# VatsalSy/gerris-fft-particles

Measured on AMD Instinct MI355X. Metric: Mcell-steps/s (projection+advection), 3D 256^3 uniform, higher is better.
Workload: dtype f64; 1 GPU; 3-D periodic Taylor-Green, 256^3 per GPU, default projection/advection parameters (SURVEY 8d config C); relax_mode=exact, parallelism=1 box, rccl_world_size=0

## Files before the change

### gerris-fft-particles_amd/csrc/domain.hip

```cpp
#include "gfship_internal.hpp"

namespace gfship {

static thread_local char g_error[1024] = "";

void set_error (const char * fmt, ...)
{
  va_list ap;
  va_start (ap, fmt);
  vsnprintf (g_error, sizeof (g_error), fmt, ap);
  va_end (ap);
}

int hip_fail (hipError_t e, const char * what, const char * file, int line)
{
  set_error ("HIP error %d (%s) in %s at %s:%d", (int) e, hipGetErrorString (e), what, file, line);
  return e == hipErrorOutOfMemory ? GFSHIP_ENOMEM : GFSHIP_EHIP;
}

Field * get_field (gfship_domain * dom, gfship_field f)
{
  if (!dom || f < 0 || (size_t) f >= dom->fields.size () || !dom->fields[f].used) {
    set_error ("invalid field handle %d", f);
    return nullptr;
// ... 162 lines not shown
  dom->gather_ctx = ctx;
  dom->lat_rank = rank; dom->lat_n = nboxes;
  for (int c = 0; c < 3; c++) dom->lat_b[c] = lattice[c];
  return GFSHIP_OK;
}

int gfship_domain_path_counts (gfship_domain * dom, unsigned long long * lattice_cycles,
			       unsigned long long * fused_mpi_launches)
{
  GFSHIP_CHECK (dom != nullptr, GFSHIP_EINVAL, "null domain");
  if (lattice_cycles) *lattice_cycles = dom->n_lattice_cycles;
  if (fused_mpi_launches) *fused_mpi_launches = dom->n_fused_mpi;
  return GFSHIP_OK;
}

int gfship_domain_kernel_counts (gfship_domain * dom, unsigned long long * counts, int n)
{
  GFSHIP_CHECK (dom != nullptr && counts != nullptr && n >= 0, GFSHIP_EINVAL, "null argument");
  for (int k = 0; k < n && k < GFSHIP_KC_COUNT; k++)
    counts[k] = dom->kc[k];
  return GFSHIP_OK;
}

int gfship_domain_synchronize (gfship_domain * dom)
{
  GFSHIP_CHECK (dom != nullptr, GFSHIP_EINVAL, "null domain");
  GFSHIP_HIP (hipStreamSynchronize (dom->stream));
  return GFSHIP_OK;
}

// ... 177 lines not shown
```

### gerris-fft-particles_amd/csrc/gfship_internal.hpp

```cpp
#pragma once

#include <hip/hip_runtime.h>
#include <cstdio>
#include <cstdarg>
#include <cstring>
#include <vector>
#include <deque>
#include <string>
#include <type_traits>
#include "gfship.h"
#include "switches.hpp"
#include "cell_update.hpp"

namespace gfship {

struct Layout {
  int n = 0;
  int px = 0;
  int xo = 1;
  int rows = 0;
  int dim = 3;
  long sy = 0;
  long sz = 0;
  size_t total = 0;
// ... 75 lines not shown
  size_t scratch_doubles = 0;
  double * h_pinned = nullptr;
  gfship_exchange_fn exchange = nullptr; void * exchange_ctx = nullptr;
  gfship_reduce_fn reduce = nullptr;     void * reduce_ctx = nullptr;
  bool has_external = false;
  void * comm = nullptr;
  int overlap = 0;
  int lat_rank = -1, lat_n = 0, lat_b[3] = { 1, 1, 1 };
  gfship_gather_fn gather = nullptr; void * gather_ctx = nullptr;
  double * lat_res = nullptr, * lat_xch = nullptr;
  unsigned * lat_bar = nullptr;
  size_t lat_res_doubles = 0, lat_xch_doubles = 0;
  double * gfv_send[6] = {}, * gfv_recv[6] = {};
  double src[3] = { 0., 0., 0. };
  unsigned long long n_lattice_cycles = 0, n_fused_mpi = 0;
  unsigned long long kc[GFSHIP_KC_COUNT] = {};
  bool lattice_attr_set = false;
  void * mpi_plan[GFSHIP_MAXLEVEL + 1] = {};
  gfship_field dp_cache = -1;
  int skew_resident = -1;
  int patch_resident = 0;
  bool no_fused_godunov = false;
  bool no_fused_loop = false;
  bool force_hyperplane = false;
  bool unit_weights = false;
  bool weighted = false;
  unsigned long weights_stamp = 0;
  gfship_field wf[6] = {-1, -1, -1, -1, -1, -1};
  gfship::SkewPlan skew[GFSHIP_MAXLEVEL + 1];
  double diff_w[GFSHIP_MAXLEVEL + 1] = {};
// ... 106 lines not shown
			   double * u, const double * rhs, const double * dia);
int launch_residual (gfship_domain * dom, int level, const double * u, const double * rhs,
		     const double * dia, double * res);
int launch_residual_weighted (gfship_domain * dom, int level, const double * u, const double * rhs,
			      const double * dia, double * res);
int launch_poisson_weights (gfship_domain * dom, double * const alpha[3]);
int launch_diffusion_weights (gfship_domain * dom, double * const D[3], double cdt);
int alloc_weights (gfship_domain * dom);
RelaxOp weighted_op (gfship_domain * dom, int level);
int launch_restrict (gfship_domain * dom, unsigned dimension, int level_coarse, double * v_coarse,
		     const double * v_fine);
int launch_prolongate (gfship_domain * dom, int level_coarse, const double * v_coarse,
		       double * v_fine);
int launch_correct (gfship_domain * dom, int level, double * u, const double * dp);
int launch_fill (gfship_domain * dom, int level, double * a, double value);
int launch_residual_norm (gfship_domain * dom, int level, const double * u, const double * rhs,
			  const double * dia, double * res, double scale, double weight,
			  double * out , bool dia_zero = false);
int launch_norm_async (gfship_domain * dom, int level, const double * a, double scale, double weight);
int launch_norm (gfship_domain * dom, int level, const double * a, double scale, double weight,
		 double out[5] );

int launch_face_interp_un (gfship_domain * dom, double * const u[3], double * const un[3]);
int launch_divergence (gfship_domain * dom, double * const un[3], double * div, double dt);
int launch_correct_un (gfship_domain * dom, const double * p, double * const un[3], double dt);
int launch_centered_gradient (gfship_domain * dom, const double * p, double * const g[3]);
int launch_correct_centered (gfship_domain * dom, double * const u[3], double * const g[3], double dt);
int launch_correct_centered_coarse (gfship_domain * dom, double * const u[3], double * const g[3],
				    double dt, double * const uc[3]);
int launch_coarse_init_from (gfship_domain * dom, Field * const * v, int nf, int top);
int launch_coarse_init_levels (gfship_domain * dom, Field * const * v, int nf, int top, int bottom);
int launch_advected_face_values (gfship_domain * dom, const double * v, double * const u[3],
				 double * const un[3], double dt, int use_centered, int gradient,
// ... 81 lines not shown
```

### gerris-fft-particles_amd/csrc/poisson.hip

```cpp
#include "gfship_internal.hpp"
#include <cmath>
#include <cfloat>
#include <cstdlib>

using namespace gfship;

namespace gfship {

static bool weighted_pipelinable (gfship_domain * dom, unsigned dimension, int level)
{
  return dom->relax_mode == GFSHIP_RELAX_EXACT && dimension == 3 && dom->dim == 3 &&
    skew_supported (dom, level) && !dom->force_hyperplane;
}

static bool weighted_pipelined (gfship_domain * dom, unsigned dimension, int level)
{
  return dom->sw.weighted_pipelined && weighted_pipelinable (dom, dimension, level);
}

static int relax_level (gfship_domain * dom, unsigned dimension, int level, double omega,
			Field * u, Field * rhs, Field * dia)
{
  u->zero[level] = false;
  if (dom->weighted) {
// ... 383 lines not shown
extern "C" {

int gfship_poisson_cycle (gfship_domain * dom, gfship_multilevel_params * p,
			  gfship_field u, gfship_field rhs, gfship_field dia, gfship_field res)
{
  GFSHIP_CHECK (dom != nullptr, GFSHIP_EINVAL, "null domain");
  int r = before_write (dom);
  if (r) return r;
  return poisson_cycle (dom, p, u, rhs, dia, res, 1., nullptr);
}

int gfship_poisson_solve (gfship_domain * dom, gfship_multilevel_params * par,
			  gfship_field lhs, gfship_field rhs, gfship_field res,
			  gfship_field dia, double dt)
{
  GFSHIP_CHECK (dom && par, GFSHIP_EINVAL, "null argument");
  Field * U = get_field (dom, lhs), * R = get_field (dom, rhs), * D = get_field (dom, dia),
    * S = get_field (dom, res);
  if (!U || !R || !D || !S) return GFSHIP_EINVAL;
  GFSHIP_CHECK (dom->unit_weights, GFSHIP_EINVAL, "call gfship_poisson_coefficients first");
  { int r = before_write (dom); if (r) return r; }
  int r;
  const int L = dom->depth;
  if ((r = coarse_flush (dom, U, L, true))) return r;
  unsigned minlevel = par->minlevel;
  par->depth = L;
  par->niter = 0;

  bool deferred = par->nitermin >= 1 && par->nitermax >= 1;
  if (deferred) {
    const Layout & Ly = dom->lay[L];
    double size = 1./Ly.n;
    S->zero[L] = false;
    if (dom->weighted) {
      if ((r = launch_residual_weighted (dom, L, U->lev[L], R->lev[L], D->lev[L], S->lev[L]))) return r;
      if ((r = launch_norm_async (dom, L, S->lev[L], 1.*size*size, 1.))) return r;
    }
    else if ((r = launch_residual_norm (dom, L, U->lev[L], R->lev[L], D->lev[L], S->lev[L], 1.*size*size,
					1., nullptr, D->zero[L])))
      return r;
  }
  else {
    if ((r = residual_and_norm (dom, dt, U, R, D, S, &par->residual))) return r;
    par->residual_before = par->residual;
  }

  double res_max_before = par->residual.infty;

  while (par->niter < par->nitermin ||
	 (par->residual.infty > par->tolerance && par->niter < par->nitermax)) {
    if ((r = poisson_cycle (dom, par, lhs, rhs, dia, res, dt, &par->residual))) {
      if (deferred) {
	deferred = false;
	double s0[5];
	if (hipStreamSynchronize (dom->stream) == hipSuccess) {
	  memcpy (s0, dom->h_pinned + 8, sizeof (s0));
	  if (norm_residual_finish (dom, dt, s0, &par->residual_before) == GFSHIP_OK)
	    par->residual = par->residual_before;
	}
	else
// ... 13 lines not shown
      break;
    if (par->residual.infty > res_max_before/1.1 && par->minlevel < par->depth)
      par->minlevel++;
    res_max_before = par->residual.infty;
    par->niter++;
  }

  par->minlevel = minlevel;
  if (r == GFSHIP_OK)
    r = skew_check_error (dom);
  if (r == GFSHIP_OK)
    r = lattice_check_error (dom);
  return r;
}

int gfship_time_relax (gfship_domain * dom, unsigned d, int level, gfship_field u,
		       gfship_field rhs, gfship_field dia, int reps, double * ms_per_sweep)
{
  Field * U = get_field (dom, u), * R = get_field (dom, rhs), * D = get_field (dom, dia);
  if (!U || !R || !D || !ms_per_sweep || reps <= 0) return GFSHIP_EINVAL;
  GFSHIP_CHECK (level >= 0 && level <= dom->depth, GFSHIP_EINVAL, "level %d out of range", level);
  int r;
  if (dom->relax_mode == GFSHIP_RELAX_EXACT && d == 3 && skew_supported (dom, level) &&
      !dom->force_hyperplane) {
    U->zero[level] = false;
    r = skew_time_sweeps (dom, level, U, R->lev[level], D->lev[level], D->zero[level], reps,
			  ms_per_sweep);
    if (r == GFSHIP_OK && dom->sw.skew_stats)
      skew_dump_stats (dom, level);
    return r;
// ... 43 lines not shown
```

### gerris-fft-particles_amd/csrc/poisson_kernels.hip

```cpp
#include "gfship_internal.hpp"
#include "cell_loop.hpp"
#include "relax_skew.hpp"
#include <algorithm>
#include <cstdlib>

namespace gfship {

template <int DIM, int OP>
__device__ __forceinline__ double relax_value (const double * __restrict__ u, long c, long sy, long sz,
					       double rhs, double dia, unsigned dimension,
					       double omega, double w, double h2, const W6 * wf = nullptr)
{
  return cell_update<DIM, OP> (kind_weights<OP> (w, ArrayW { wf, c }), ArrayU { u, c, sy, sz }, rhs, dia, u + c,
			       dimension, omega, h2);
}

__device__ __forceinline__ double relax_value_six (const double * __restrict__ u, long c, long sy, long sz,
						    double rhs)
{
  return cell_update_six (ArrayU { u, c, sy, sz }, rhs);
}

template <int DIM, int OP>
__global__ void __launch_bounds__(256)
// ... 1036 lines not shown
  }
  GFSHIP_HIP (hipGetLastError ());
  return GFSHIP_OK;
}

template <int DIM>
__global__ void __launch_bounds__(256)
residual_kernel (Layout L, const double * __restrict__ u, const double * __restrict__ rhs,
		 const double * __restrict__ dia, double * __restrict__ res)
{
  CELL_LOOP_PROLOGUE (L);
  const FaceSums s = face_sums<DIM> (UnitW {}, ArrayU { u, c, L.sy, L.sz }, dia[c]);
  res[c] = residual_close (s.a, s.b, rhs[c], u[c]);
}

template <bool NORM>
__global__ void residual_norm2_kernel (Layout L, const double * __restrict__ u, const double * __restrict__ rhs,
				       const double * __restrict__ dia, double * __restrict__ res, double inv,
				       double weight, double * __restrict__ partial);

int launch_residual (gfship_domain * dom, int level, const double * u, const double * rhs,
		     const double * dia, double * res)
{
  const Layout & L = dom->lay[level];
  dim3 grid, block;
  cell_grid (L, &grid, &block);
  const bool pairs = dom->sw.residual_pairs;
  if (dom->dim == 3 && L.n >= 64) dom->kc[pairs ? GFSHIP_KC_RESIDUAL_PAIRS : GFSHIP_KC_RESIDUAL_SCALAR]++;
  if (dom->dim == 3 && L.n >= 64 && pairs) {
    const long nitems = (long) L.n*L.n*(L.n/2);
    long nb = (nitems + 255)/256;
    if (nb > 4096) nb = 4096;
    hipLaunchKernelGGL (residual_norm2_kernel<false>, dim3 ((int) nb), dim3 (256), 0, dom->stream, L, u, rhs,
			dia, res, 1., 1., nullptr);
    GFSHIP_HIP (hipGetLastError ());
    return GFSHIP_OK;
  }
  with_bools ([&] (auto D3) {
    hipLaunchKernelGGL (residual_kernel<decltype (D3)::value ? 3 : 2>, grid, block, 0, dom->stream, L, u, rhs, dia, res);
  }, dom->dim == 3);
  GFSHIP_HIP (hipGetLastError ());
  return GFSHIP_OK;
}

template <int DIM>
__global__ void __launch_bounds__(256)
residual_weighted_kernel (Layout L, const double * __restrict__ u, const double * __restrict__ rhs,
			  const double * __restrict__ dia, double * __restrict__ res, W6 wf)
{
// ... 383 lines not shown
      const FaceSums f = face_sums<DIM> (UnitW {}, ArrayU { u, c, L.sy, L.sz }, dia ? dia[c] : 0.);
      const double raw = residual_close (f.a, f.b, rhs[c], u[c]);
      res[c] = raw;
      double val = raw*inv;
      s0 += weight*val;
      val = fabs (val);
      s3 = fmax (s3, val);
      s1 += weight*val;
      s2 += weight*val*val;
      s4 += raw;
    }
  }
  block_norm_sums (s0, s1, s2, s3, s4, partial, blockIdx.x);
}

template <bool NORM>
__global__ void __launch_bounds__(256)
residual_norm2_kernel (Layout L, const double * __restrict__ u, const double * __restrict__ rhs,
		       const double * __restrict__ dia, double * __restrict__ res, double inv,
		       double weight, double * __restrict__ partial)
{
  typedef double d2 __attribute__((ext_vector_type(2)));
  const int n = L.n, half = n >> 1;
  const long nitems = (long) n*n*half;
  double s0 = 0., s1 = 0., s2 = 0., s3 = 0., s4 = 0.;
  for (long it = (long) blockIdx.x*blockDim.x + threadIdx.x; it < nitems; it += (long) gridDim.x*blockDim.x) {
    const int pr = (int) (it % half);
    const long r = it / half;
    const int j = (int) (r % n) + 1, k = (int) (r / n) + 1;
    const long c = L.idx (1 + 2*pr, j, k);
    const d2 uc = *(const d2 *) (u + c);
    const double ul = u[c - 1], ur = u[c + 2];
    const d2 ut = *(const d2 *) (u + c + L.sy), ub = *(const d2 *) (u + c - L.sy);
    const d2 uf = *(const d2 *) (u + c + L.sz), uk = *(const d2 *) (u + c - L.sz);
    const d2 rh = *(const d2 *) (rhs + c);
// ... 9 lines not shown
      a += 1.; b += 1.*uf.x;
      a += 1.; b += 1.*uk.x;
      out.x = rh.x - (b - uc.x*a);
    }
    {
      double a = di.y, b = 0.;
      a += 1.; b += 1.*ur;
      a += 1.; b += 1.*uc.x;
      a += 1.; b += 1.*ut.y;
      a += 1.; b += 1.*ub.y;
      a += 1.; b += 1.*uf.y;
      a += 1.; b += 1.*uk.y;
      out.y = rh.y - (b - uc.y*a);
    }
    *(d2 *) (res + c) = out;
    if (NORM)
#pragma unroll
    for (int e = 0; e < 2; e++) {
      const double raw = e ? out.y : out.x;
      double val = raw*inv;
      s0 += weight*val;
      val = fabs (val);
      s3 = fmax (s3, val);
      s1 += weight*val;
      s2 += weight*val*val;
      s4 += raw;
    }
  }
  if (!NORM) return;
  __shared__ double sh[5][4];
// ... 2 lines not shown
  if (lane == 0) { sh[0][w] = s0; sh[1][w] = s1; sh[2][w] = s2; sh[3][w] = s3; sh[4][w] = s4; }
  __syncthreads ();
  if (threadIdx.x == 0) {
    int nw = blockDim.x >> 6;
    double r0 = 0., r1 = 0., r2 = 0., r3 = 0., r4 = 0.;
    for (int q = 0; q < nw; q++) {
      r0 += sh[0][q]; r1 += sh[1][q]; r2 += sh[2][q]; r3 = fmax (r3, sh[3][q]); r4 += sh[4][q];
    }
    double * p = partial + 5*(size_t) blockIdx.x;
    p[0] = r0; p[1] = r1; p[2] = r2; p[3] = r3; p[4] = r4;
  }
}

int launch_residual_norm (gfship_domain * dom, int level, const double * u, const double * rhs,
			  const double * dia, double * res, double scale, double weight,
			  double * out, bool dia_zero)
{
  const Layout & L = dom->lay[level];
  if (!power_of_two (scale)) {
    int r = launch_residual (dom, level, u, rhs, dia, res);
    if (r) return r;
    return out ? launch_norm (dom, level, res, scale, weight, out) :
      launch_norm_async (dom, level, res, scale, weight);
  }
  long nrows = L.dim == 3 ? (long) L.n*L.n : L.n;
  int block = L.n >= 256 ? 256 : L.n >= 128 ? 128 : 64;
  int rn_blocks = dom->sw.rn_blocks;
  if (rn_blocks < 64 || rn_blocks > 8192) rn_blocks = 4096;
  int nblocks = (int) (nrows > rn_blocks ? rn_blocks : nrows);
  double * partial = dom->d_scratch;
  double * result = out ? dom->h_pinned : dom->h_pinned + 8;
  const bool rn_pairs = dom->sw.residual_pairs;
  if (dom->dim == 3 && L.n >= 64) dom->kc[rn_pairs ? GFSHIP_KC_RESIDUAL_PAIRS : GFSHIP_KC_RESIDUAL_SCALAR]++;
  if (dom->dim == 3 && L.n >= 64 && rn_pairs) {
    const long nitems = (long) L.n*L.n*(L.n/2);
    long nb = (nitems + 255)/256;
    nblocks = (int) (nb > rn_blocks ? rn_blocks : nb);
    hipLaunchKernelGGL (residual_norm2_kernel<true>, dim3 (nblocks), dim3 (256), 0, dom->stream, L, u,
			rhs, dia_zero ? nullptr : dia, res, 1./scale, weight, partial);
  }
  else
    with_bools ([&] (auto D3) {
      hipLaunchKernelGGL (residual_norm_kernel<decltype (D3)::value ? 3 : 2>, dim3 (nblocks), dim3 (block), 0,
			  dom->stream, L, u, rhs, dia_zero ? nullptr : dia, res, 1./scale, weight, partial);
    }, dom->dim == 3);
  hipLaunchKernelGGL (norm_final_kernel, dim3 (1), dim3 (256), 0, dom->stream,
		      partial, nblocks, result);
  GFSHIP_HIP (hipGetLastError ());
  dom->kc[GFSHIP_KC_RN_BLOCKS_LIMIT] = rn_blocks;
  if ((unsigned long long) nblocks > dom->kc[GFSHIP_KC_RN_BLOCKS_MAX])
    dom->kc[GFSHIP_KC_RN_BLOCKS_MAX] = nblocks;
  if (out) {
    GFSHIP_HIP (stream_wait_spin (dom->stream));
    memcpy (out, dom->h_pinned, 5*sizeof (double));
// ... 159 lines not shown
```

### gerris-fft-particles_amd/csrc/simulation.hip

```cpp
#include "gfship_internal.hpp"
#include <cmath>
#include <cfloat>
#include <cstdlib>

using namespace gfship;

#define G_MAXINT 2147483647

struct gfship_sim {
  gfship_domain * dom = nullptr;
  gfship_field p = -1, pmac = -1, u[3] = {-1, -1, -1}, g[3] = {-1, -1, -1}, gmac[3] = {-1, -1, -1};
  std::vector<gfship_field> tracers;
  std::vector<int> tracer_gradient;
  gfship_field un[3] = {-1, -1, -1};
  gfship_field fv[6] = {-1, -1, -1, -1, -1, -1};
  gfship_field dia = -1, div = -1, res = -1, tmp = -1;
  gfship_multilevel_params projection_params, approx_projection_params;
  gfship_advection_params advection_params;
  double t = 0., end = DBL_MAX, dtmax = DBL_MAX, tnext = 0.;
  unsigned i = 0, iend = G_MAXINT;
  double visc[3] = {0., 0., 0.};
  gfship_field alpha[3] = {-1, -1, -1};
  bool has_alpha = false;
  gfship_field viscf[3][3] = {{-1, -1, -1}, {-1, -1, -1}, {-1, -1, -1}};
// ... 120 lines not shown
}

int materialize_un (gfship_sim * s)
{
  if (!s->un_lazy) return GFSHIP_OK;
  s->un_lazy = false;
  double * uold[3], * un[3];
  ptrs3 (s, s->adv_tmp3, uold);
  ptrs3 (s, s->un, un);
  TRY (launch_face_interp_un (s->dom, uold, un));
  TRY (launch_correct_un (s->dom, leaf (s, s->p), un, s->un_lazy_dt));
  return GFSHIP_OK;
}

int mac_projection (gfship_sim * s, gfship_multilevel_params * par, double dt, gfship_field p,
		    const gfship_field g[3], bool approximate = false, bool lazy = false)
{
  gfship_domain * dom = s->dom;
  double * un[3], * gp[3], * u[3];
  ptrs3 (s, s->un, un);
  ptrs3 (s, g, gp);
  ptrs3 (s, s->u, u);
  if (s->has_alpha) {
    TRY (gfship_poisson_coefficients_alpha (dom, s->alpha));
    lazy = false;
  }
  else
    TRY (gfship_poisson_coefficients (dom));
  for (int l = 0; l <= dom->depth; l++)
    if (!dom->fields[s->dia].zero[l])
      TRY (gfship_field_fill (dom, s->dia, l, 0.));
// ... 2 lines not shown
  if (!approximate || !s->tracers.empty () || s->un_handle_given || p != s->p || !dom->sw.lazy_un)
    lazy = false;
  if (!approximate)
    TRY (materialize_un (s));
  else
    s->un_lazy = false;
  if (approximate)
    TRY (launch_face_interp_div (dom, u, lazy ? nullptr : un, leaf (s, s->div), dt));
  else if (!(s->div_ready && s->div_dt == dt)) {
    TRY (launch_divergence (dom, un, leaf (s, s->div), dt));
    dom->kc[GFSHIP_KC_DIVERGENCE_SEPARATE]++;
  }
  else
    dom->kc[GFSHIP_KC_DIVERGENCE_FUSED]++;
  s->div_ready = false;
  TRY (gfship_poisson_solve (dom, par, p, s->div, s->res, s->dia, dt));
  s->cfl_ready = false;
  bool want_max = approximate, ghosts_done = false;
  for (int c = 0; c < dom->dim; c++)
    if (has_viscosity (s, c) || dom->src[c] != 0. || s->has_srcf) want_max = false;
  if (s->has_alpha) {
    want_max = false;
    TRY (launch_project_correct_weighted (dom, leaf (s, p), un, gp, approximate ? u : nullptr, dt));
  }
  else if (lazy) {
    const int L = dom->depth;
    double * uo[3];
    for (int c = 0; c < dom->dim; c++) {
      if (s->adv_tmp3[c] < 0)
	s->adv_tmp3[c] = gfship_field_alloc (dom, -1);
      if (s->adv_tmp3[c] < 0) return s->adv_tmp3[c];
// ... 671 lines not shown
    v.push_back (get_field (dom, s->u[c]));
  for (gfship_field t : s->tracers)
    v.push_back (get_field (dom, t));
}

int gfship_sim_set_tracer_gradient (gfship_sim * s, int t, int gradient)
{
  GFSHIP_CHECK (s != nullptr, GFSHIP_EINVAL, "null simulation");
  GFSHIP_CHECK (t >= 0 && (size_t) t < s->tracers.size (), GFSHIP_EINVAL, "no tracer %d", t);
  GFSHIP_CHECK (gradient >= 0 && gradient <= 4, GFSHIP_EINVAL,
		"gradient: 0 centred, 1 van Leer, 2 minmod, 3 superbee, 4 sweby");
  s->tracer_gradient[t] = gradient;
  return GFSHIP_OK;
}

static int coarse_init (gfship_sim * s, bool u_done);

int gfship_coarse_init (gfship_sim * s)
{
  GFSHIP_CHECK (s != nullptr, GFSHIP_EINVAL, "null simulation");
  return coarse_init (s, false);
}

static int coarse_init (gfship_sim * s, bool u_done)
{
  std::vector<Field *> v;
  sim_variables (s, v);
  Field * pmac = get_field (s->dom, s->pmac);
  std::vector<Field *> now, vel;
  for (Field * F : v) {
    bool is_u = false;
    for (int c = 0; c < s->dom->dim; c++)
      if (F == get_field (s->dom, s->u[c])) is_u = true;
    if (F == pmac) F->coarse_stale = true;
    else {
      F->coarse_stale = false;
      F->coarse_valid = true;
      if (u_done && is_u) vel.push_back (F); else now.push_back (F);
    }
  }
  if (vel.empty ())
    return launch_coarse_init (s->dom, now.data (), (int) now.size ());
  TRY (launch_coarse_init_levels (s->dom, now.data (), (int) now.size (), s->dom->depth - 1, s->dom->depth - 1));
  now.insert (now.end (), vel.begin (), vel.end ());
  if (s->dom->depth >= 2)
    TRY (launch_coarse_init_levels (s->dom, now.data (), (int) now.size (), s->dom->depth - 2, 0));
  return GFSHIP_OK;
}

int gfship_sim_start (gfship_sim * s)
{
  GFSHIP_CHECK (s != nullptr, GFSHIP_EINVAL, "null simulation");
  GFSHIP_CHECK (s->advection_params.gc, GFSHIP_EUNSUPPORTED, "gc = 0 is not supported");
  TRY (bc_leaf (s, s->p));
  TRY (bc_leaf (s, s->pmac));
// ... 57 lines not shown

  {
    Field * P = get_field (dom, s->p), * PM = get_field (dom, s->pmac);
    std::swap (P->lev, PM->lev);
    int r = mac_projection (s, &s->projection_params, s->advection_params.dt/2., s->p, s->gmac);
    std::swap (P->lev, PM->lev);
    if (r != GFSHIP_OK) return r;
  }

  bool u_coarse = false, corrected = false;
  TRY (centered_velocity_advection (s, s->gmac, s->i > 0 ? gc : s->gmac, - s->advection_params.dt,
				    &corrected, &u_coarse));
  if (!corrected)
    TRY (correct_centered_velocities (s, s->i > 0 ? gc : s->gmac, - s->advection_params.dt, &u_coarse));

  TRY (coarse_init (s, u_coarse));

  TRY (mac_projection (s, &s->approx_projection_params, s->advection_params.dt, s->p, s->g, true, true));
  s->t = s->tnext;
  s->i++;

  TRY (set_timestep (s, true));
  TRY (advance_tracers (s, s->advection_params.dt));
  return GFSHIP_OK;
}

int gfship_divergence_norm (gfship_sim * s, gfship_norm * out)
{
  GFSHIP_CHECK (s && out, GFSHIP_EINVAL, "null argument");
  double * u[3];
  ptrs3 (s, s->u, u);
  TRY (launch_velocity_divergence (s->dom, u, leaf (s, s->div)));
  return gfship_norm_variable (s->dom, s->div, out);
// ... 12 lines not shown
```

### gerris-fft-particles_amd/csrc/timestep_kernels.hip

```cpp
#include "gfship_internal.hpp"
#include "cell_loop.hpp"
#include <cfloat>

namespace gfship {

#define EXT_PROLOGUE(L)							\
  int i = blockIdx.x*blockDim.x + threadIdx.x;				\
  int j = blockIdx.y;							\
  int k = (L).dim == 3 ? blockIdx.z : 0;				\
  if (i > (L).n) return;						\
  long c = (L).idx (i, j, k)

static inline void ext_grid (const Layout & L, dim3 * grid, dim3 * block)
{
  int b = L.n >= 256 ? 256 : L.n >= 128 ? 128 : 64;
  *block = dim3 (b);
  *grid = dim3 ((L.n + 1 + b - 1)/b, L.n + 1, L.dim == 3 ? L.n + 1 : 1);
}

struct Ptr3  { double * p[3]; };
struct CPtr3 { const double * p[3]; };
struct Ptr6  { double * p[6]; };
struct CPtr6 { const double * p[6]; };
struct Visc3 { double d[3]; double g[3]; };
// ... 2527 lines not shown
  for (int f = 0; f < A.nf; f++) {
    double val = 0., sa = 0.;
#pragma unroll
    for (int id = 0; id < (1 << DIM); id++) {
      int ci = 2*i - 1 + (id & 1);
      int cj = 2*j - 1 + ((id & 2) ? 0 : 1);
      int ck = DIM == 3 ? 2*k - 1 + ((id & 4) ? 0 : 1) : 0;
      double a = 1.;
      val += A.vf[f][Lf.idx (ci, cj, ck)]*a;
      sa += a;
    }
    A.vc[f][c] = val/sa;
  }
}

template <int DIM>
__global__ void __launch_bounds__(256)
velocity_divergence_kernel (Layout L, CPtr3 u, double * __restrict__ out)
{
  CELL_LOOP_PROLOGUE (L);
  const long off[3] = { 1, L.sy, L.sz };
  double h = 1./L.n;
  double div = 0.;
#pragma unroll
  for (int cc = 0; cc < DIM; cc++) {
    div += 1.*1.*face_interp (u.p[cc][c], u.p[cc][c + off[cc]]);
    div += 1.*-1.*face_interp (u.p[cc][c], u.p[cc][c - off[cc]]);
  }
  out[c] = div/(1.*h);
}
// ... 481 lines not shown

int launch_coarse_init (gfship_domain * dom, Field * const * v, int nf)
{
  return launch_coarse_init_from (dom, v, nf, dom->depth - 1);
}

int launch_coarse_init_from (gfship_domain * dom, Field * const * v, int nf, int top)
{
  return launch_coarse_init_levels (dom, v, nf, top, 0);
}

int launch_coarse_init_levels (gfship_domain * dom, Field * const * v, int nf, int top, int bottom)
{
  for (int f0 = 0; f0 < nf; f0 += 8) {
    int m = nf - f0 < 8 ? nf - f0 : 8;
    for (int l = top; l >= bottom; l--) {
      const Layout & Lc = dom->lay[l], & Lf = dom->lay[l + 1];
      CoarseArgs A;
      A.nf = m;
      for (int f = 0; f < m; f++) {
	A.vc[f] = v[f0 + f]->lev[l];
	A.vf[f] = v[f0 + f]->lev[l + 1];
	v[f0 + f]->zero[l] = false;
	v[f0 + f]->coarse_valid = true;
      }
      dim3 grid, block;
      cell_grid (Lc, &grid, &block);
      DISPATCH (dom, coarse_init_kernel, grid, block, Lc, Lf, A);
    }
  }
  return GFSHIP_OK;
}

int launch_velocity_divergence (gfship_domain * dom, double * const u[3], double * out)
{
  const Layout & L = dom->lay[dom->depth];
  dim3 grid, block;
  cell_grid (L, &grid, &block);
  DISPATCH (dom, velocity_divergence_kernel, grid, block, L, c3 (u), out);
  return GFSHIP_OK;
}

}
```

### gerris-fft-particles_amd/gfship/__init__.py

```python
import ctypes as C
import os
import sys

import numpy as np

_PKG = os.path.dirname(os.path.dirname(os.path.abspath(__file__)))
LIB_PATH = os.environ.get("GFSHIP_LIB", os.path.join(_PKG, "lib", "libgfship.so"))

SIDE_PERIODIC, SIDE_BOUNDARY, SIDE_EXTERNAL = 0, 1, 2
BC_SYMMETRY, BC_DIRICHLET, BC_NEUMANN = 0, 1, 2
RELAX_EXACT, RELAX_REDBLACK, RELAX_EXACT_HYPERPLANE, RELAX_EXACT_PER_SWEEP = 0, 1, 2, 3


class GfshipError(RuntimeError):
    pass


class Norm(C.Structure):
    _fields_ = [("bias", C.c_double), ("first", C.c_double), ("second", C.c_double),
                ("infty", C.c_double), ("w", C.c_double)]


class MultilevelParams(C.Structure):
    _fields_ = [("tolerance", C.c_double), ("nrelax", C.c_uint), ("erelax", C.c_uint),
# ... 29 lines not shown
    "gfship_field_download": (_i, [_vp, _i, _i, _pd]),
    "gfship_field_fill": (_i, [_vp, _i, _i, _d]),
    "gfship_field_device_ptr": (_vp, [_vp, _i, _i, _pi, _pi]),
    "gfship_bc": (_i, [_vp, _i, _i, _i]),
    "gfship_homogeneous_bc": (_i, [_vp, _i, _i, _i]),
    "gfship_multilevel_params_init": (None, [C.POINTER(MultilevelParams), _i]),
    "gfship_poisson_coefficients": (_i, [_vp]),
    "gfship_poisson_coefficients_alpha": (_i, [_vp, _pi]),
    "gfship_poisson_weights": (_i, [_vp, _i, _pi]),
    "gfship_relax": (_i, [_vp, _u, _i, _d, _i, _i, _i]),
    "gfship_residual": (_i, [_vp, _u, _i, _i, _i, _i, _i]),
    "gfship_norm_residual": (_i, [_vp, _d, _i, C.POINTER(Norm)]),
    "gfship_norm_variable": (_i, [_vp, _i, C.POINTER(Norm)]),
    "gfship_poisson_cycle": (_i, [_vp, C.POINTER(MultilevelParams), _i, _i, _i, _i]),
    "gfship_poisson_solve": (_i, [_vp, C.POINTER(MultilevelParams), _i, _i, _i, _i, _d]),
    "gfship_diffusion_coefficients": (_i, [_vp, _d, _d, _i, _d]),
    "gfship_diffusion_coefficients_faces": (_i, [_vp, _pi, _d, _i, _i, _d]),
    "gfship_diffusion_rhs": (_i, [_vp, _i, _i, _i, _d]),
    "gfship_diffusion_residual": (_i, [_vp, _i, _i, _i, _i]),
    "gfship_diffusion_cycle": (_i, [_vp, _u, _u, _u, _i, _i, _i, _i]),
    "gfship_diffusion": (_i, [_vp, C.POINTER(MultilevelParams), _i, _i, _i]),
    "gfship_time_relax": (_i, [_vp, _u, _i, _i, _i, _i, _i, _pd]),
    "gfship_time_relax_loop": (_i, [_vp, _i, _i, _i, _i, _u, _i, _pd, _pi]),
    "gfship_time_relax_loop_inclusive": (_i, [_vp, _i, _i, _i, _i, _u, _i, _pd, _pi, _pd]),
    "gfship_sim_create": (_i, [C.POINTER(_vp), _vp]),
    "gfship_sim_destroy": (None, [_vp]),
    "gfship_sim_variable": (_i, [_vp, _i, _i]),
    "gfship_sim_projection_params": (C.POINTER(MultilevelParams), [_vp]),
    "gfship_sim_approx_projection_params": (C.POINTER(MultilevelParams), [_vp]),
    "gfship_sim_advection_params": (C.POINTER(AdvectionParams), [_vp]),
# ... 19 lines not shown
    "gfship_approximate_projection": (_i, [_vp, C.POINTER(MultilevelParams), _d, _i, _pi]),
    "gfship_centered_velocity_advection": (_i, [_vp, _pi, _pi]),
    "gfship_correct_centered_velocities": (_i, [_vp, _pi, _d]),
    "gfship_sim_advance_time": (_i, [_vp]),
    "gfship_tracer_advection": (_i, [_vp, _i, _d]),
    "gfship_domain_cfl": (_i, [_vp, _pd]),
    "gfship_set_timestep": (_i, [_vp]),
    "gfship_coarse_init": (_i, [_vp]),
    "gfship_divergence_norm": (_i, [_vp, C.POINTER(Norm)]),
    "gfship_sim_download_un": (_i, [_vp, _i, _pd]),
    "gfship_domain_set_overlap": (_i, [_vp, _i]),
    "gfship_domain_set_exchange": (_i, [_vp, _vp, _vp]),
    "gfship_domain_set_reduce": (_i, [_vp, _vp, _vp]),
    "gfship_domain_set_gather": (_i, [_vp, _vp, _vp, _i, _i, C.POINTER(C.c_int)]),
    "gfship_domain_path_counts": (_i, [_vp, C.POINTER(C.c_ulonglong), C.POINTER(C.c_ulonglong)]),
    "gfship_domain_kernel_counts": (_i, [_vp, C.POINTER(C.c_ulonglong), _i]),
    "gfship_sim_restart": (_i, [_vp, _d, _u]),
    "gfship_snapshot_tree_bytes": (C.c_size_t, [_vp, _i]),
    "gfship_snapshot_tree_write": (_i, [_vp, _i, _pi, _vp, C.c_size_t]),
    "gfship_snapshot_tree_read": (_i, [_vp, _i, _pi, _vp, C.c_size_t]),
    "gfship_comm_available": (_i, []),
    "gfship_comm_unique_id": (_i, [_vp]),
    "gfship_domain_comm_init": (_i, [_vp, _vp, _i, _i, _pi]),
    "gfship_domain_comm_size": (_i, [_vp]),
    "gfship_domain_comm_stats": (_i, [_vp, C.POINTER(C.c_ulonglong), C.POINTER(C.c_ulonglong)]),
    "gfship_domain_comm_destroy": (_i, [_vp]),
    "gfship_halo_pack": (_i, [_vp, _vp, _i, _i, _vp]),
    "gfship_halo_unpack": (_i, [_vp, _vp, _i, _i, _vp]),
    "gfship_halo_pack_sides": (_i, [_vp, _vp, _i, _i, _pi, C.POINTER(_vp)]),
    "gfship_halo_unpack_sides": (_i, [_vp, _vp, _i, _i, _pi, C.POINTER(_vp)]),
# ... 177 lines not shown
        _check(lib().gfship_domain_comm_init(self.ptr, buf, rank, nranks, (C.c_int * 3)(*lattice)))

    def comm_size(self):
        return _check(lib().gfship_domain_comm_size(self.ptr))

    def comm_stats(self):
        m, b = C.c_ulonglong(), C.c_ulonglong()
        _check(lib().gfship_domain_comm_stats(self.ptr, C.byref(m), C.byref(b)))
        return int(m.value), int(b.value)

    def path_counts(self):
        a, b = C.c_ulonglong(), C.c_ulonglong()
        _check(lib().gfship_domain_path_counts(self.ptr, C.byref(a), C.byref(b)))
        return int(a.value), int(b.value)

    def kernel_counts(self):
        n = len(KERNEL_COUNT_NAMES)
        a = (C.c_ulonglong * n)()
        _check(lib().gfship_domain_kernel_counts(self.ptr, a, n))
        return {name: int(a[k]) for k, name in enumerate(KERNEL_COUNT_NAMES)}

    def snapshot_tree(self, variables):
        n = len(variables)
        h = (C.c_int * n)(*[v.h for v in variables])
        size = lib().gfship_snapshot_tree_bytes(self.ptr, n)
        buf = C.create_string_buffer(size)
        _check(lib().gfship_snapshot_tree_write(self.ptr, n, h, buf, size))
        return buf.raw

    def snapshot_tree_read(self, variables, data):
# ... 46 lines not shown
    def norm_residual(self, res, dt=1.):
        n = Norm()
        _check(lib().gfship_norm_residual(self.ptr, dt, res.h, C.byref(n)))
        return n

    def norm_variable(self, v):
        n = Norm()
        _check(lib().gfship_norm_variable(self.ptr, v.h, C.byref(n)))
        return n

    def poisson_cycle(self, par, u, rhs, dia, res):
        _check(lib().gfship_poisson_cycle(self.ptr, C.byref(par), u.h, rhs.h, dia.h, res.h))

    def poisson_solve(self, par, lhs, rhs, res, dia, dt=1.):
        _check(lib().gfship_poisson_solve(self.ptr, C.byref(par), lhs.h, rhs.h, res.h, dia.h, dt))

    def diffusion_coefficients(self, D, dt, rhoc, beta=1.):
        _check(lib().gfship_diffusion_coefficients(self.ptr, D, dt, rhoc.h, beta))

    def diffusion_coefficients_faces(self, D, dt, rhoc, alpha_cell=None, beta=1.):
        h = (C.c_int * 3)(*([v.h for v in D] + [-1] * (3 - len(D))))
        _check(lib().gfship_diffusion_coefficients_faces(self.ptr, h, dt, rhoc.h,
                                                         -1 if alpha_cell is None else alpha_cell.h, beta))

    def diffusion_rhs(self, v, rhs, rhoc, beta=1.):
        _check(lib().gfship_diffusion_rhs(self.ptr, v.h, rhs.h, rhoc.h, beta))

    def diffusion_residual(self, u, rhs, rhoc, res):
        _check(lib().gfship_diffusion_residual(self.ptr, u.h, rhs.h, rhoc.h, res.h))

# ... 502 lines not shown
```

### include/gfship.h

```cpp
#ifndef GFSHIP_H
#define GFSHIP_H

#include <stddef.h>

#ifdef __cplusplus
extern "C" {
#endif

#define GFSHIP_VERSION   1
#define GFSHIP_MAXLEVEL  12

enum { GFSHIP_OK = 0, GFSHIP_EINVAL = -1, GFSHIP_ENODEVICE = -2, GFSHIP_ENOMEM = -3,
       GFSHIP_EHIP = -4, GFSHIP_EUNSUPPORTED = -5 };

enum { GFSHIP_SIDE_PERIODIC = 0,
       GFSHIP_SIDE_BOUNDARY = 1,
       GFSHIP_SIDE_EXTERNAL = 2 };

enum { GFSHIP_BC_SYMMETRY = 0, GFSHIP_BC_DIRICHLET = 1, GFSHIP_BC_NEUMANN = 2 };

enum { GFSHIP_RELAX_EXACT = 0, GFSHIP_RELAX_REDBLACK = 1, GFSHIP_RELAX_EXACT_HYPERPLANE = 2,
       GFSHIP_RELAX_EXACT_PER_SWEEP = 3 };

typedef struct gfship_domain gfship_domain;
// ... 45 lines not shown
void gfship_multilevel_params_init (gfship_multilevel_params * par, int dim);
int  gfship_poisson_coefficients (gfship_domain * dom);
int  gfship_poisson_coefficients_alpha (gfship_domain * dom, const gfship_field alpha[3]);
int  gfship_poisson_weights (gfship_domain * dom, int d, gfship_field * w);
int  gfship_relax (gfship_domain * dom, unsigned d, int level, double omega,
		   gfship_field u, gfship_field rhs, gfship_field dia);
int  gfship_residual (gfship_domain * dom, unsigned d, int level,
		      gfship_field u, gfship_field rhs, gfship_field dia, gfship_field res);
int  gfship_norm_residual (gfship_domain * dom, double dt, gfship_field res, gfship_norm * out);
int  gfship_norm_variable (gfship_domain * dom, gfship_field v, gfship_norm * out);
int  gfship_poisson_cycle (gfship_domain * dom, gfship_multilevel_params * p,
			   gfship_field u, gfship_field rhs, gfship_field dia, gfship_field res);
int  gfship_poisson_solve (gfship_domain * dom, gfship_multilevel_params * par,
			   gfship_field lhs, gfship_field rhs, gfship_field res,
			   gfship_field dia, double dt);


int  gfship_diffusion_coefficients (gfship_domain * dom, double D, double dt, gfship_field rhoc,
				    double beta);
int  gfship_diffusion_coefficients_faces (gfship_domain * dom, const gfship_field D[3], double dt,
					  gfship_field rhoc, gfship_field alpha_cell, double beta);
int  gfship_diffusion_rhs (gfship_domain * dom, gfship_field v, gfship_field rhs,
			   gfship_field rhoc, double beta);
int  gfship_diffusion_residual (gfship_domain * dom, gfship_field u, gfship_field rhs,
				gfship_field rhoc, gfship_field res);
int  gfship_diffusion_cycle (gfship_domain * dom, unsigned levelmin, unsigned depth,
			     unsigned nrelax, gfship_field u, gfship_field rhs, gfship_field rhoc,
			     gfship_field res);
int  gfship_diffusion (gfship_domain * dom, gfship_multilevel_params * par, gfship_field v,
		       gfship_field rhs, gfship_field rhoc);
// ... 174 lines not shown
  GFSHIP_KC_PATCH_LOOP_KERNEL_ARMS,
  GFSHIP_KC_PATCH_LOOP_HOST_ARMS,
  GFSHIP_KC_XCD_SCOPE_ON,
  GFSHIP_KC_XCD_SCOPE_OFF,
  GFSHIP_KC_XCD_NEAR_MODE,
  GFSHIP_KC_XCD_PLACE_ON,
  GFSHIP_KC_XCD_PLACE_OFF,
  GFSHIP_KC_COARSE_CYCLES,
  GFSHIP_KC_COARSE_THREADS,
  GFSHIP_KC_COARSE_END_BY_LEVEL,
  GFSHIP_KC_DIFFUSION_FACES_PIPELINED,
  GFSHIP_KC_DIFFUSION_FACES_HYPERPLANES,
  GFSHIP_KC_COUNT
};
int  gfship_domain_kernel_counts (gfship_domain * dom, unsigned long long * counts, int n);
#define GFSHIP_UNIQUE_ID_BYTES 128
int  gfship_comm_available (void);
int  gfship_comm_unique_id (void * id);
int  gfship_domain_comm_init (gfship_domain * dom, const void * unique_id, int rank, int nranks,
			      const int lattice[3]);
int  gfship_domain_comm_size (gfship_domain * dom);
int  gfship_domain_comm_stats (gfship_domain * dom, unsigned long long * messages,
			       unsigned long long * bytes);
int  gfship_domain_comm_destroy (gfship_domain * dom);

int  gfship_halo_pack (gfship_domain * dom, const void * dev_ptr, int level, int side, void * dev_buf);
int  gfship_halo_unpack (gfship_domain * dom, void * dev_ptr, int level, int side, const void * dev_buf);
int  gfship_halo_pack_sides (gfship_domain * dom, const void * dev_ptr, int level, int nsides,
			     const int * sides, void * const * dev_bufs);
int  gfship_halo_unpack_sides (gfship_domain * dom, void * dev_ptr, int level, int nsides,
// ... 62 lines not shown
```

Baseline: 2694 Mcell-steps/s.

## Fuse pressure restriction into residual kernel and batch small coarse levels

Has the final residual/norm pass of the approximate projection solve also write the 8-cell average of the finest pressure into the next-coarser level, so the full-resolution coarse-init restriction of P no longer needs its own read of the fine field. The remaining coarse levels and other fields are restricted afterwards. Adds a single-block kernel that restricts all levels of size 8 and smaller in one launch instead of one launch per level. This cuts a full-grid memory pass and several small kernel launches per step, at the cost of reordering coarse_init relative to the projection and adding code paths with new on/off switches.

```diff
diff --git a/gerris-fft-particles_amd/csrc/domain.hip b/gerris-fft-particles_amd/csrc/domain.hip
--- a/gerris-fft-particles_amd/csrc/domain.hip
+++ b/gerris-fft-particles_amd/csrc/domain.hip
@@ -200,6 +200,23 @@
   return GFSHIP_OK;
 }
 
+int gfship_domain_set_coarse_paths (gfship_domain * dom, int residual_coarse, int small_levels)
+{
+  GFSHIP_CHECK (dom != nullptr, GFSHIP_EINVAL, "null domain");
+  dom->no_residual_coarse = !residual_coarse;
+  dom->no_small_coarse_levels = !small_levels;
+  return GFSHIP_OK;
+}
+
+int gfship_domain_residual_coarse_counts (gfship_domain * dom, unsigned long long * fused,
+					  unsigned long long * declined)
+{
+  GFSHIP_CHECK (dom != nullptr, GFSHIP_EINVAL, "null domain");
+  if (fused) *fused = dom->n_residual_coarse;
+  if (declined) *declined = dom->n_residual_coarse_declined;
+  return GFSHIP_OK;
+}
+
 int gfship_domain_kernel_counts (gfship_domain * dom, unsigned long long * counts, int n)
 {
   GFSHIP_CHECK (dom != nullptr && counts != nullptr && n >= 0, GFSHIP_EINVAL, "null argument");
diff --git a/gerris-fft-particles_amd/csrc/gfship_internal.hpp b/gerris-fft-particles_amd/csrc/gfship_internal.hpp
--- a/gerris-fft-particles_amd/csrc/gfship_internal.hpp
+++ b/gerris-fft-particles_amd/csrc/gfship_internal.hpp
@@ -113,6 +113,9 @@
   double * gfv_send[6] = {}, * gfv_recv[6] = {};
   double src[3] = { 0., 0., 0. };
   unsigned long long n_lattice_cycles = 0, n_fused_mpi = 0;
+  unsigned long long n_residual_coarse = 0, n_residual_coarse_declined = 0;
+  bool no_residual_coarse = false;
+  bool no_small_coarse_levels = false;
   unsigned long long kc[GFSHIP_KC_COUNT] = {};
   bool lattice_attr_set = false;
   void * mpi_plan[GFSHIP_MAXLEVEL + 1] = {};
@@ -249,9 +252,35 @@
 		       double * v_fine);
 int launch_correct (gfship_domain * dom, int level, double * u, const double * dp);
 int launch_fill (gfship_domain * dom, int level, double * a, double value);
+struct ResidualExtras {
+  double * coarse = nullptr;
+  bool coarse_done = false;
+};
 int launch_residual_norm (gfship_domain * dom, int level, const double * u, const double * rhs,
 			  const double * dia, double * res, double scale, double weight,
-			  double * out , bool dia_zero = false);
+			  double * out , bool dia_zero = false,
+			  ResidualExtras * x = nullptr);
+inline bool residual_coarse_applies (const gfship_domain * dom, int level)
+{
+  return dom->dim == 3 && level >= 1 && !dom->weighted && dom->lay[level].n >= 64 && dom->sw.residual_pairs &&
+    !dom->no_residual_coarse;
+}
+inline bool solve_residual_is_pair_pass (const gfship_domain * dom, const gfship_multilevel_params * par)
+{
+  return par->nitermin >= 1 && par->nitermax >= 1 && dom->dim == 3 && !dom->weighted &&
+    dom->lay[dom->depth].n >= 64 && dom->sw.residual_pairs;
+}
+inline bool solve_leaves_coarse (const gfship_domain * dom, const gfship_multilevel_params * par)
+{
+  return solve_residual_is_pair_pass (dom, par) && residual_coarse_applies (dom, dom->depth);
+}
+struct CoarseRequest {
+  Field * const * fields = nullptr;
+  int nf = 0;
+  bool done = false;
+};
+int poisson_solve (gfship_domain * dom, gfship_multilevel_params * par, gfship_field lhs, gfship_field rhs,
+		   gfship_field res, gfship_field dia, double dt, CoarseRequest * coarse);
 int launch_norm_async (gfship_domain * dom, int level, const double * a, double scale, double weight);
 int launch_norm (gfship_domain * dom, int level, const double * a, double scale, double weight,
 		 double out[5] );
diff --git a/gerris-fft-particles_amd/csrc/poisson.hip b/gerris-fft-particles_amd/csrc/poisson.hip
--- a/gerris-fft-particles_amd/csrc/poisson.hip
+++ b/gerris-fft-particles_amd/csrc/poisson.hip
@@ -421,6 +421,31 @@
 			  gfship_field lhs, gfship_field rhs, gfship_field res,
 			  gfship_field dia, double dt)
 {
+  return gfship::poisson_solve (dom, par, lhs, rhs, res, dia, dt, nullptr);
+}
+
+int gfship_poisson_solve_coarse (gfship_domain * dom, gfship_multilevel_params * par,
+				 gfship_field lhs, gfship_field rhs, gfship_field res,
+				 gfship_field dia, double dt, int * coarse_done)
+{
+  GFSHIP_CHECK (dom && coarse_done, GFSHIP_EINVAL, "null argument");
+  Field * U = get_field (dom, lhs);
+  if (!U) return GFSHIP_EINVAL;
+  Field * one[1] = { U };
+  CoarseRequest cr;
+  cr.fields = one;
+  cr.nf = 1;
+  int r = gfship::poisson_solve (dom, par, lhs, rhs, res, dia, dt, &cr);
+  *coarse_done = cr.done;
+  return r;
+}
+
+}
+
+int gfship::poisson_solve (gfship_domain * dom, gfship_multilevel_params * par,
+			   gfship_field lhs, gfship_field rhs, gfship_field res,
+			   gfship_field dia, double dt, CoarseRequest * coarse)
+{
   GFSHIP_CHECK (dom && par, GFSHIP_EINVAL, "null argument");
   Field * U = get_field (dom, lhs), * R = get_field (dom, rhs), * D = get_field (dom, dia),
     * S = get_field (dom, res);
@@ -435,6 +460,7 @@
   par->niter = 0;
 
   bool deferred = par->nitermin >= 1 && par->nitermax >= 1;
+  if (coarse) coarse->done = false;
   if (deferred) {
     const Layout & Ly = dom->lay[L];
     double size = 1./Ly.n;
@@ -443,14 +469,27 @@
       if ((r = launch_residual_weighted (dom, L, U->lev[L], R->lev[L], D->lev[L], S->lev[L]))) return r;
       if ((r = launch_norm_async (dom, L, S->lev[L], 1.*size*size, 1.))) return r;
     }
-    else if ((r = launch_residual_norm (dom, L, U->lev[L], R->lev[L], D->lev[L], S->lev[L], 1.*size*size,
-					1., nullptr, D->zero[L])))
-      return r;
+    else {
+      ResidualExtras x;
+      if (coarse && L >= 1 && solve_leaves_coarse (dom, par))
+	x.coarse = U->lev[L - 1];
+      if ((r = launch_residual_norm (dom, L, U->lev[L], R->lev[L], D->lev[L], S->lev[L], 1.*size*size,
+				     1., nullptr, D->zero[L], &x)))
+	return r;
+      if (x.coarse_done) {
+	coarse->done = true;
+	U->zero[L - 1] = false;
+	U->coarse_valid = true;
+	if (L >= 2 && (r = launch_coarse_init_levels (dom, coarse->fields, coarse->nf, L - 2, 0))) return r;
+      }
+    }
   }
   else {
     if ((r = residual_and_norm (dom, dt, U, R, D, S, &par->residual))) return r;
     par->residual_before = par->residual;
   }
+  if (coarse)
+    (coarse->done ? dom->n_residual_coarse : dom->n_residual_coarse_declined)++;
 
   double res_max_before = par->residual.infty;
 
@@ -494,6 +533,8 @@
   return r;
 }
 
+extern "C" {
+
 int gfship_time_relax (gfship_domain * dom, unsigned d, int level, gfship_field u,
 		       gfship_field rhs, gfship_field dia, int reps, double * ms_per_sweep)
 {
diff --git a/gerris-fft-particles_amd/csrc/poisson_kernels.hip b/gerris-fft-particles_amd/csrc/poisson_kernels.hip
--- a/gerris-fft-particles_amd/csrc/poisson_kernels.hip
+++ b/gerris-fft-particles_amd/csrc/poisson_kernels.hip
@@ -1074,10 +1074,11 @@
   res[c] = residual_close (s.a, s.b, rhs[c], u[c]);
 }
 
-template <bool NORM>
+template <bool NORM, bool COARSE = false>
 __global__ void residual_norm2_kernel (Layout L, const double * __restrict__ u, const double * __restrict__ rhs,
 				       const double * __restrict__ dia, double * __restrict__ res, double inv,
-				       double weight, double * __restrict__ partial);
+				       double weight, double * __restrict__ partial, Layout Lc,
+				       double * __restrict__ ucoarse);
 
 int launch_residual (gfship_domain * dom, int level, const double * u, const double * rhs,
 		     const double * dia, double * res)
@@ -1092,7 +1093,7 @@
     long nb = (nitems + 255)/256;
     if (nb > 4096) nb = 4096;
     hipLaunchKernelGGL (residual_norm2_kernel<false>, dim3 ((int) nb), dim3 (256), 0, dom->stream, L, u, rhs,
-			dia, res, 1., 1., nullptr);
+			dia, res, 1., 1., nullptr, Layout (), nullptr);
     GFSHIP_HIP (hipGetLastError ());
     return GFSHIP_OK;
   }
@@ -1506,11 +1507,11 @@
   block_norm_sums (s0, s1, s2, s3, s4, partial, blockIdx.x);
 }
 
-template <bool NORM>
+template <bool NORM, bool COARSE>
 __global__ void __launch_bounds__(256)
 residual_norm2_kernel (Layout L, const double * __restrict__ u, const double * __restrict__ rhs,
 		       const double * __restrict__ dia, double * __restrict__ res, double inv,
-		       double weight, double * __restrict__ partial)
+		       double weight, double * __restrict__ partial, Layout Lc, double * __restrict__ ucoarse)
 {
   typedef double d2 __attribute__((ext_vector_type(2)));
   const int n = L.n, half = n >> 1;
@@ -1550,6 +1551,15 @@
       out.y = rh.y - (b - uc.y*a);
     }
     *(d2 *) (res + c) = out;
+    if (COARSE && (j & 1) && (k & 1)) {
+      const d2 uq = *(const d2 *) (u + c + L.sy + L.sz);
+      double val = 0.;
+      val += uq.x; val += uq.y;
+      val += uf.x; val += uf.y;
+      val += ut.x; val += ut.y;
+      val += uc.x; val += uc.y;
+      ucoarse[Lc.idx (pr + 1, (j + 1) >> 1, (k + 1) >> 1)] = val/8.;
+    }
     if (NORM)
 #pragma unroll
     for (int e = 0; e < 2; e++) {
@@ -1582,9 +1592,10 @@
 
 int launch_residual_norm (gfship_domain * dom, int level, const double * u, const double * rhs,
 			  const double * dia, double * res, double scale, double weight,
-			  double * out, bool dia_zero)
+			  double * out, bool dia_zero, ResidualExtras * x)
 {
   const Layout & L = dom->lay[level];
+  if (x) x->coarse_done = false;
   if (!power_of_two (scale)) {
     int r = launch_residual (dom, level, u, rhs, dia, res);
     if (r) return r;
@@ -1604,8 +1615,13 @@
     const long nitems = (long) L.n*L.n*(L.n/2);
     long nb = (nitems + 255)/256;
     nblocks = (int) (nb > rn_blocks ? rn_blocks : nb);
-    hipLaunchKernelGGL (residual_norm2_kernel<true>, dim3 (nblocks), dim3 (256), 0, dom->stream, L, u,
-			rhs, dia_zero ? nullptr : dia, res, 1./scale, weight, partial);
+    const bool coarse = x && x->coarse && residual_coarse_applies (dom, level);
+    with_bools ([&] (auto C) {
+      hipLaunchKernelGGL ((residual_norm2_kernel<true, decltype (C)::value>), dim3 (nblocks), dim3 (256), 0,
+			  dom->stream, L, u, rhs, dia_zero ? nullptr : dia, res, 1./scale, weight, partial,
+			  coarse ? dom->lay[level - 1] : Layout (), coarse ? x->coarse : nullptr);
+    }, coarse);
+    if (x) x->coarse_done = coarse;
   }
   else
     with_bools ([&] (auto D3) {
diff --git a/gerris-fft-particles_amd/csrc/simulation.hip b/gerris-fft-particles_amd/csrc/simulation.hip
--- a/gerris-fft-particles_amd/csrc/simulation.hip
+++ b/gerris-fft-particles_amd/csrc/simulation.hip
@@ -158,7 +158,8 @@
 }
 
 int mac_projection (gfship_sim * s, gfship_multilevel_params * par, double dt, gfship_field p,
-		    const gfship_field g[3], bool approximate = false, bool lazy = false)
+		    const gfship_field g[3], bool approximate = false, bool lazy = false,
+		    CoarseRequest * coarse = nullptr)
 {
   gfship_domain * dom = s->dom;
   double * un[3], * gp[3], * u[3];
@@ -191,7 +192,7 @@
   else
     dom->kc[GFSHIP_KC_DIVERGENCE_FUSED]++;
   s->div_ready = false;
-  TRY (gfship_poisson_solve (dom, par, p, s->div, s->res, s->dia, dt));
+  TRY (poisson_solve (dom, par, p, s->div, s->res, s->dia, dt, coarse));
   s->cfl_ready = false;
   bool want_max = approximate, ghosts_done = false;
   for (int c = 0; c < dom->dim; c++)
@@ -893,7 +894,7 @@
   return GFSHIP_OK;
 }
 
-static int coarse_init (gfship_sim * s, bool u_done);
+static int coarse_init (gfship_sim * s, bool u_done, std::vector<Field *> * later = nullptr);
 
 int gfship_coarse_init (gfship_sim * s)
 {
@@ -901,7 +902,7 @@
   return coarse_init (s, false);
 }
 
-static int coarse_init (gfship_sim * s, bool u_done)
+static int coarse_init (gfship_sim * s, bool u_done, std::vector<Field *> * later)
 {
   std::vector<Field *> v;
   sim_variables (s, v);
@@ -918,6 +919,17 @@
       if (u_done && is_u) vel.push_back (F); else now.push_back (F);
     }
   }
+  if (later) {
+    Field * P = get_field (s->dom, s->p);
+    std::vector<Field *> rest;
+    for (Field * F : now)
+      if (F != P) rest.push_back (F);
+    if (!rest.empty ())
+      TRY (launch_coarse_init_levels (s->dom, rest.data (), (int) rest.size (), s->dom->depth - 1, s->dom->depth - 1));
+    *later = now;
+    later->insert (later->end (), vel.begin (), vel.end ());
+    return GFSHIP_OK;
+  }
   if (vel.empty ())
     return launch_coarse_init (s->dom, now.data (), (int) now.size ());
   TRY (launch_coarse_init_levels (s->dom, now.data (), (int) now.size (), s->dom->depth - 1, s->dom->depth - 1));
@@ -1005,9 +1017,19 @@
   if (!corrected)
     TRY (correct_centered_velocities (s, s->i > 0 ? gc : s->gmac, - s->advection_params.dt, &u_coarse));
 
-  TRY (coarse_init (s, u_coarse));
-
-  TRY (mac_projection (s, &s->approx_projection_params, s->advection_params.dt, s->p, s->g, true, true));
+  if (!s->has_alpha && dom->depth >= 1 && solve_leaves_coarse (dom, &s->approx_projection_params)) {
+    std::vector<Field *> later;
+    TRY (coarse_init (s, u_coarse, &later));
+    CoarseRequest cr;
+    cr.fields = later.data ();
+    cr.nf = (int) later.size ();
+    TRY (mac_projection (s, &s->approx_projection_params, s->advection_params.dt, s->p, s->g, true, true, &cr));
+    GFSHIP_CHECK (cr.done, GFSHIP_EUNSUPPORTED, "the solve did not leave the coarse cells of P it was asked for");
+  }
+  else {
+    TRY (coarse_init (s, u_coarse));
+    TRY (mac_projection (s, &s->approx_projection_params, s->advection_params.dt, s->p, s->g, true, true));
+  }
   s->t = s->tnext;
   s->i++;
 
diff --git a/gerris-fft-particles_amd/csrc/timestep_kernels.hip b/gerris-fft-particles_amd/csrc/timestep_kernels.hip
--- a/gerris-fft-particles_amd/csrc/timestep_kernels.hip
+++ b/gerris-fft-particles_amd/csrc/timestep_kernels.hip
@@ -2565,6 +2565,33 @@
   }
 }
 
+struct CoarseSmallArgs { double * lev[8][5]; Layout lay[5]; int nf, top, bottom; };
+
+__global__ void __launch_bounds__(1024)
+coarse_init_small_kernel (CoarseSmallArgs A)
+{
+  typedef double d2 __attribute__((ext_vector_type(2)));
+  for (int l = A.top; l >= A.bottom; l--) {
+    const Layout Lc = A.lay[l], Lf = A.lay[l + 1];
+    const int nc = 1 << (3*l), m = (1 << l) - 1;
+    for (int q = threadIdx.x; q < nc*A.nf; q += blockDim.x) {
+      const int f = q >> (3*l), cc = q & (nc - 1);
+      const int i = (cc & m) + 1, j = ((cc >> l) & m) + 1, k = (cc >> (2*l)) + 1;
+      const double * vf = A.lev[f][l + 1] + Lf.idx (2*i - 1, 2*j - 1, 2*k - 1);
+      const d2 a = *(const d2 *) (vf + Lf.sy + Lf.sz), b = *(const d2 *) (vf + Lf.sz);
+      const d2 c = *(const d2 *) (vf + Lf.sy), d = *(const d2 *) vf;
+      double val = 0.;
+      val += a.x; val += a.y;
+      val += b.x; val += b.y;
+      val += c.x; val += c.y;
+      val += d.x; val += d.y;
+      A.lev[f][l][Lc.idx (i, j, k)] = val/8.;
+    }
+    __threadfence_block ();
+    __syncthreads ();
+  }
+}
+
 template <int DIM>
 __global__ void __launch_bounds__(256)
 velocity_divergence_kernel (Layout L, CPtr3 u, double * __restrict__ out)
@@ -3076,7 +3103,14 @@
 {
   for (int f0 = 0; f0 < nf; f0 += 8) {
     int m = nf - f0 < 8 ? nf - f0 : 8;
-    for (int l = top; l >= bottom; l--) {
+    int stop = -1;
+    if (dom->dim == 3 && !dom->no_small_coarse_levels) {
+      stop = top < 3 ? top : 3;
+      while (stop >= 0 && dom->lay[stop].n > 8) stop--;
+      if (stop - bottom < 1 || dom->lay[stop].n != 1 << stop) stop = -1;
+    }
+    const int per_level_bottom = stop >= 0 ? stop + 1 : bottom;
+    for (int l = top; l >= per_level_bottom; l--) {
       const Layout & Lc = dom->lay[l], & Lf = dom->lay[l + 1];
       CoarseArgs A;
       A.nf = m;
@@ -3090,6 +3124,22 @@
       cell_grid (Lc, &grid, &block);
       DISPATCH (dom, coarse_init_kernel, grid, block, Lc, Lf, A);
     }
+    if (stop >= 0) {
+      CoarseSmallArgs A;
+      A.nf = m; A.top = stop; A.bottom = bottom;
+      for (int l = 0; l <= stop + 1; l++) {
+	A.lay[l] = dom->lay[l];
+	for (int f = 0; f < m; f++)
+	  A.lev[f][l] = v[f0 + f]->lev[l];
+      }
+      for (int f = 0; f < m; f++) {
+	for (int l = bottom; l <= stop; l++)
+	  v[f0 + f]->zero[l] = false;
+	v[f0 + f]->coarse_valid = true;
+      }
+      hipLaunchKernelGGL (coarse_init_small_kernel, dim3 (1), dim3 (1024), 0, dom->stream, A);
+      GFSHIP_HIP (hipGetLastError ());
+    }
   }
   return GFSHIP_OK;
 }
diff --git a/gerris-fft-particles_amd/gfship/__init__.py b/gerris-fft-particles_amd/gfship/__init__.py
--- a/gerris-fft-particles_amd/gfship/__init__.py
+++ b/gerris-fft-particles_amd/gfship/__init__.py
@@ -67,6 +67,7 @@
     "gfship_norm_variable": (_i, [_vp, _i, C.POINTER(Norm)]),
     "gfship_poisson_cycle": (_i, [_vp, C.POINTER(MultilevelParams), _i, _i, _i, _i]),
     "gfship_poisson_solve": (_i, [_vp, C.POINTER(MultilevelParams), _i, _i, _i, _i, _d]),
+    "gfship_poisson_solve_coarse": (_i, [_vp, C.POINTER(MultilevelParams), _i, _i, _i, _i, _d, C.POINTER(C.c_int)]),
     "gfship_diffusion_coefficients": (_i, [_vp, _d, _d, _i, _d]),
     "gfship_diffusion_coefficients_faces": (_i, [_vp, _pi, _d, _i, _i, _d]),
     "gfship_diffusion_rhs": (_i, [_vp, _i, _i, _i, _d]),
@@ -116,6 +117,8 @@
     "gfship_domain_set_reduce": (_i, [_vp, _vp, _vp]),
     "gfship_domain_set_gather": (_i, [_vp, _vp, _vp, _i, _i, C.POINTER(C.c_int)]),
     "gfship_domain_path_counts": (_i, [_vp, C.POINTER(C.c_ulonglong), C.POINTER(C.c_ulonglong)]),
+    "gfship_domain_set_coarse_paths": (_i, [_vp, _i, _i]),
+    "gfship_domain_residual_coarse_counts": (_i, [_vp, C.POINTER(C.c_ulonglong), C.POINTER(C.c_ulonglong)]),
     "gfship_domain_kernel_counts": (_i, [_vp, C.POINTER(C.c_ulonglong), _i]),
     "gfship_sim_restart": (_i, [_vp, _d, _u]),
     "gfship_snapshot_tree_bytes": (C.c_size_t, [_vp, _i]),
@@ -323,6 +326,14 @@
         _check(lib().gfship_domain_path_counts(self.ptr, C.byref(a), C.byref(b)))
         return int(a.value), int(b.value)
 
+    def set_coarse_paths(self, residual_coarse=True, small_levels=True):
+        _check(lib().gfship_domain_set_coarse_paths(self.ptr, int(bool(residual_coarse)), int(bool(small_levels))))
+
+    def residual_coarse_counts(self):
+        a, b = C.c_ulonglong(), C.c_ulonglong()
+        _check(lib().gfship_domain_residual_coarse_counts(self.ptr, C.byref(a), C.byref(b)))
+        return int(a.value), int(b.value)
+
     def kernel_counts(self):
         n = len(KERNEL_COUNT_NAMES)
         a = (C.c_ulonglong * n)()
@@ -399,6 +410,12 @@
 
     def poisson_solve(self, par, lhs, rhs, res, dia, dt=1.):
         _check(lib().gfship_poisson_solve(self.ptr, C.byref(par), lhs.h, rhs.h, res.h, dia.h, dt))
+
+    def poisson_solve_coarse(self, par, lhs, rhs, res, dia, dt=1.):
+        done = C.c_int(0)
+        _check(lib().gfship_poisson_solve_coarse(self.ptr, C.byref(par), lhs.h, rhs.h, res.h, dia.h, dt,
+                                                 C.byref(done)))
+        return bool(done.value)
 
     def diffusion_coefficients(self, D, dt, rhoc, beta=1.):
         _check(lib().gfship_diffusion_coefficients(self.ptr, D, dt, rhoc.h, beta))
diff --git a/include/gfship.h b/include/gfship.h
--- a/include/gfship.h
+++ b/include/gfship.h
@@ -83,6 +83,9 @@
 int  gfship_poisson_solve (gfship_domain * dom, gfship_multilevel_params * par,
 			   gfship_field lhs, gfship_field rhs, gfship_field res,
 			   gfship_field dia, double dt);
+int  gfship_poisson_solve_coarse (gfship_domain * dom, gfship_multilevel_params * par,
+				  gfship_field lhs, gfship_field rhs, gfship_field res,
+				  gfship_field dia, double dt, int * coarse_done);
 
 
 int  gfship_diffusion_coefficients (gfship_domain * dom, double D, double dt, gfship_field rhoc,
@@ -287,6 +290,9 @@
   GFSHIP_KC_COUNT
 };
 int  gfship_domain_kernel_counts (gfship_domain * dom, unsigned long long * counts, int n);
+int  gfship_domain_set_coarse_paths (gfship_domain * dom, int residual_coarse, int small_levels);
+int  gfship_domain_residual_coarse_counts (gfship_domain * dom, unsigned long long * fused,
+					   unsigned long long * declined);
 #define GFSHIP_UNIQUE_ID_BYTES 128
 int  gfship_comm_available (void);
 int  gfship_comm_unique_id (void * id);
```

Result: no change. 2706 Mcell-steps/s (median of 5 runs) (+0.4%).
